# huzjkevin/planar_optical_flow

Measured on AMD Instinct MI355X. Metric: scans/sec, flow-only preprocess of 450-pt synthetic scan pairs, batch 4096 per GPU (+ flow EPE vs reference oracle), higher is better.
Workload: dtype f32 flow arithmetic (float32 outputs) + f64 exact association / mask decisions; the float64-output instantiation (the reference's float64 operation order) is `value_f64`

## Files before the change

planar_optical_flow_amd/csrc/scan_flow.hip:

```cpp
#include <cmath>
#include <cstdlib>
#include <type_traits>

#include "pof_common.h"

namespace {

constexpr int kThreads = 256;

__global__ void laser_phi_kernel(double start, double stop, double step, int n, double *tab)
{
    int i = blockIdx.x * blockDim.x + threadIdx.x;
    if (i >= n) return;
    double p = (double)i * step;
    p = p + start;
    if (i == n - 1 && n > 1) p = stop;
    double s, c;
    sincos(p, &s, &c);
    tab[i] = p;
    tab[n + 2 * i] = c;
    tab[n + 2 * i + 1] = s;
}

struct PreArgs {
    const float *ranges;
    long long sample_stride;
    int B, N, D;
    const double *tab;
    const double *odom0, *odom1;
    int flow_kind, canonical;
    void *xy, *flow;
    const int32_t *det_offsets;
    const double *det_rphi;
    const uint8_t *det_cls;
    double ra0, ra1, ra2;
    double sd0, sd1, sd2;
    double sa0, sa1, sa2;
    int32_t lb0, lb1, lb2;
    int64_t *closest, *target_cls;
    float *target_reg, *dyn_mask, *valid_mask, *exclude_mask;
    double *ws_rec;
    double *ws_det;
};

constexpr int kDetStride = 6;
constexpr int kInline = 8;
constexpr int kRecImg = 8 + kInline * kDetStride;
constexpr int kRecHdrFloats = 16;
constexpr int kImgScreen = kRecHdrFloats * 4;
constexpr int kImgCtr = kImgScreen + 16 * kInline;
constexpr int kImgMot = kImgCtr + 16 * kInline;
constexpr int kImgBytes = kImgMot + 64;
constexpr int kRecStride = kRecImg + kImgBytes / 8;

__device__ __forceinline__ double opaque_zero()
{
    double z;
    asm volatile("v_mov_b64 %0, 0" : "=v"(z));
    return z;
}

__device__ __forceinline__ void motion_params(int kind, const double *o0, const double *o1, double sA, double cA,
                              double sB, double cB, double *mot)
{
    const double tx = o1[0] - o0[0], ty = o1[1] - o0[1];
    if (kind == 0) {
        const float c0 = (float)cA, s0 = (float)sA, c1 = (float)cB, s1 = (float)sB;
        const float p00 = fmaf(s0, s1, c0 * c1);
        const float p01 = fmaf(s0, c1, c0 * (-s1));
        const float p10 = fmaf(c0, s1, (-s0) * c1);
        const float p11 = fmaf(c0, c1, (-s0) * (-s1));
        mot[0] = 1.0 - (double)p00;
        mot[1] = 0.0 - (double)p01;
        mot[2] = 0.0 - (double)p10;
        mot[3] = 1.0 - (double)p11;
        mot[4] = fma((double)c0, tx, (double)s0 * ty);
        mot[5] = fma((double)(-s0), tx, (double)c0 * ty);
        mot[6] = opaque_zero();
    } else if (kind == 1) {
        mot[0] = cB; mot[1] = -sB; mot[2] = sB; mot[3] = cB;
        mot[4] = fma(ty, -sA, tx * cA);
        mot[5] = fma(ty, cA, tx * sA);
        mot[6] = opaque_zero();
    } else if (kind == 2) {
        const float c1 = (float)cB, s1 = (float)sB;
        mot[0] = mot[1] = mot[2] = mot[3] = opaque_zero();
        mot[4] = fma((double)c1, tx, (double)s1 * ty);
        mot[5] = fma((double)(-s1), tx, (double)c1 * ty);
        mot[6] = o1[2] - o0[2];
    } else if (kind == 3) {
        const double dt = o1[0], den = dt + 1e-6;
        mot[0] = o0[2] / den;
        mot[1] = o0[0] / den;
        mot[2] = o0[1] / den;
        mot[3] = dt;
        mot[4] = mot[5] = mot[6] = opaque_zero();
    } else {
        const float c = (float)cA, sn = (float)sA, cd = (float)cB, sd = (float)sB;
        mot[0] = (double)c; mot[1] = (double)sn; mot[2] = (double)(-sn); mot[3] = (double)c;
        mot[4] = fma(o0[1], (double)(-sd), o0[0] * (double)cd);
        mot[5] = fma(o0[1], (double)cd, o0[0] * (double)sd);
        mot[6] = opaque_zero();
    }
}

__device__ __forceinline__ double motion_angle(int kind, int which, const double *o0, const double *o1)
{
    if (kind == 1) return which ? o1[2] - o0[2] : o0[2];
    if (kind == 4) return which ? o1[0] : o0[2];
    return which ? o1[2] : o0[2];
}

__device__ __forceinline__ void apply_motion(int kind, double px, double py, double m0, double m1, double m2,
                                             double m3, double t0, double t1, double dph, double &fx,
                                             double &fy)
{
    if (kind == 0) {
        fx = fma(py, m1, px * m0) - t0;
        fy = fma(py, m3, px * m2) - t1;
    } else if (kind == 1) {
        fx = (fma(py, m1, px * m0) - t0) - px;
        fy = (fma(py, m3, px * m2) - t1) - py;
    } else if (kind == 2) {
        fx = -t0 - (py * -dph);
        fy = -t1 - (px * dph);
    } else if (kind == 3) {
        fx = ((0.0 - m0 * py) + m1) * m3;
        fy = ((m0 * px - 0.0) + m2) * m3;
    } else {
        fx = fma(py, m1, px * m0) + t0;
        fy = fma(py, m3, px * m2) + t1;
    }
}

__device__ __forceinline__ double poly_sin(double x, double y)
{
    const double S1 = -1.66666666666666324348e-01, S2 = 8.33333333332248946124e-03, S3 = -1.98412698298579493134e-04,
                 S4 = 2.75573137070700676789e-06, S5 = -2.50507602534068634195e-08, S6 = 1.58969099521155010221e-10;
    const double z = x * x, v = z * x;
    const double r = S2 + z * (S3 + z * (S4 + z * (S5 + z * S6)));
    return x - ((z * (0.5 * y - v * r) - y) - v * S1);
}
__device__ __forceinline__ double poly_cos(double x, double y)
{
    const double C1 = 4.16666666666666019037e-02, C2 = -1.38888888888741095749e-03, C3 = 2.48015872894767294178e-05,
                 C4 = -2.75573143513906633035e-07, C5 = 2.08757232129817482790e-09, C6 = -1.13596475577881948265e-11;
    const double z = x * x;
    const double r = z * (C1 + z * (C2 + z * (C3 + z * (C4 + z * (C5 + z * C6)))));
    const double ax = fabs(x);
    if (ax < 0.3) return 1.0 - (0.5 * z - (z * r - x * y));
    const double qx = ax > 0.78125 ? 0.28125 : 0.25 * ax;
    const double hz = 0.5 * z - qx, a = 1.0 - qx;
    return a - (hz - (z * r - x * y));
}
template <bool FALLBACK>
__device__ __forceinline__ void params_sincos(double x, double *sn, double *cs)
{
    const double ax = fabs(x);
    if (!(ax < 823549.0)) {
        if (FALLBACK) {
            sincos(x, sn, cs);
        } else {
            *sn = *cs = __builtin_nan("");
// ... 14 lines not shown
        r = t - w;
        w = fn * p2t - ((t - r) - w);
        y0 = r - w;
        if (ex - ((__double2hiint(y0) >> 20) & 0x7ff) > 49) {
            t = r;
            w = fn * p3;
            r = t - w;
            w = fn * p3t - ((t - r) - w);
            y0 = r - w;
        }
    }
    double y1 = (r - y0) - w;
    int n = (int)fn;
    if (x < 0.0) {
        y0 = -y0;
        y1 = -y1;
        n = -n;
    }
    const double s = poly_sin(y0, y1), c = poly_cos(y0, y1);
    const bool odd = (n & 1) != 0;
    double ss = odd ? c : s, cc = odd ? s : c;
    if (n & 2) ss = -ss;
    if ((n + 1) & 2) cc = -cc;
    *sn = ss;
    *cs = cc;
}

template <typename AP>
__device__ __forceinline__ void det_entry(AP a, int g, double *w)
{
    const double dr = a->det_rphi[2 * g], dp = a->det_rphi[2 * g + 1];
    double s, c;
    sincos(dp, &s, &c);
    const int cl = a->det_cls[g];
    w[0] = dr * c;
    w[1] = dr * s;
    w[2] = cl == 0 ? a->ra0 : (cl == 1 ? a->ra1 : a->ra2);
    w[3] = cl == 0 ? a->sd0 : (cl == 1 ? a->sd1 : a->sd2);
    w[4] = (double)(cl == 0 ? a->lb0 : (cl == 1 ? a->lb1 : a->lb2));
    w[5] = cl == 0 ? a->sa0 : (cl == 1 ? a->sa1 : a->sa2);
}

__device__ __forceinline__ bool det_is_far(double cx, double cy, double sd)
{
    return !(fabs(cx) + fabs(cy) < 100.0) || !(sd <= 400.0);
}

__host__ __device__ inline int params_job_count(int B, bool have_dets)
{
    (void)have_dets;
    return kInline * B;
}

template <bool FALLBACK, bool WRITE_F64, typename AP>
__device__ __forceinline__ void params_work(AP a, int t)
{
    if (t >= kInline * a->B) return;
    const int b = t >> 3, slot = t & 7;
    double *rec = a->ws_rec + (long long)b * kRecStride;
    unsigned char *img = reinterpret_cast<unsigned char *>(rec + kRecImg);
    int d0 = 0, cnt = 0;
    if (a->det_offsets) {
        d0 = a->det_offsets[b];
        cnt = a->det_offsets[b + 1] - d0;
    }
    const int npass = 1 + (cnt - slot + kInline - 1) / kInline;
#pragma unroll 1
    for (int pass = a->flow ? 0 : 1; pass < max(npass, 1); ++pass) {
        const int idx = slot + kInline * (pass - 1);
        const bool active = pass == 0 ? slot < 2 : idx < cnt;
        double ang = 0.0, dr = 0.0;
        if (pass == 0) {
            if (active) ang = motion_angle(a->flow_kind, slot, a->odom0 + 3 * b, a->odom1 + 3 * b);
        } else if (active) {
            dr = a->det_rphi[2 * (d0 + idx)];
            ang = a->det_rphi[2 * (d0 + idx) + 1];
        }
        double sn, cs;
        params_sincos<FALLBACK>(ang, &sn, &cs);
        if (pass == 0) {
            const double s_o = __shfl_xor(sn, 1, 64), c_o = __shfl_xor(cs, 1, 64);
            if (slot == 0) {
                double *m64 = reinterpret_cast<double *>(img + kImgMot);
                motion_params(a->flow_kind, a->odom0 + 3 * b, a->odom1 + 3 * b, sn, cs, s_o, c_o, m64);
                m64[7] = (double)cnt;
                float4 *hf = reinterpret_cast<float4 *>(img);
                hf[0] = make_float4((float)m64[0], (float)m64[1], (float)m64[2], (float)m64[3]);
                hf[1] = make_float4((float)m64[4], (float)m64[5], (float)m64[6], __int_as_float(cnt));
                if (WRITE_F64) {
                    double2 *r2 = reinterpret_cast<double2 *>(rec);
#pragma unroll
                    for (int k = 0; k < 4; ++k) r2[k] = make_double2(m64[2 * k], m64[2 * k + 1]);
                }
            }
        } else if (active) {
            const unsigned cl = a->det_cls[d0 + idx] > 1 ? 2u : (unsigned)a->det_cls[d0 + idx];
            double w[kDetStride];
            w[0] = dr * cs;
            w[1] = dr * sn;
            w[2] = cl == 0 ? a->ra0 : (cl == 1 ? a->ra1 : a->ra2);
            w[3] = cl == 0 ? a->sd0 : (cl == 1 ? a->sd1 : a->sd2);
            w[4] = (double)(cl == 0 ? a->lb0 : (cl == 1 ? a->lb1 : a->lb2));
            w[5] = cl == 0 ? a->sa0 : (cl == 1 ? a->sa1 : a->sa2);
            if (idx < kInline) {
                const bool far = det_is_far(w[0], w[1], w[3]);
                reinterpret_cast<float4 *>(img + kImgScreen)[idx] =
                    make_float4((float)w[0], (float)w[1], far ? INFINITY : -(float)w[3], (float)(w[5] - w[3]));
                reinterpret_cast<double2 *>(img + kImgCtr)[idx] = make_double2(w[0], w[1]);
                img[32 + idx] = (unsigned char)cl;
                img[40 + idx] = far ? 1 : 0;
                if (WRITE_F64) {
                    double2 *r2 = reinterpret_cast<double2 *>(rec + 8 + idx * kDetStride);
                    r2[0] = make_double2(w[0], w[1]);
                    r2[1] = make_double2(w[2], w[3]);
                    r2[2] = make_double2(w[4], w[5]);
                }
            }
            if (cnt > kInline) {
                double2 *r2 = reinterpret_cast<double2 *>(a->ws_det + (long long)(d0 + idx) * kDetStride);
                r2[0] = make_double2(w[0], w[1]);
                r2[1] = make_double2(w[2], w[3]);
                r2[2] = make_double2(w[4], w[5]);
            }
        }
    }
    if (!a->flow && slot == 0) {
        reinterpret_cast<int *>(img)[7] = cnt;
        reinterpret_cast<double *>(img + kImgMot)[7] = (double)cnt;
        if (WRITE_F64) rec[7] = (double)cnt;
    }
    if (a->det_offsets && slot >= cnt) {
        reinterpret_cast<float4 *>(img + kImgScreen)[slot] = make_float4(0.0f, 0.0f, INFINITY, 0.0f);
        img[40 + slot] = 0;
    }
}

__global__ __launch_bounds__(256) void scan_params_kernel(PreArgs a)
{
    params_work<true, true>(&a, blockIdx.x * blockDim.x + threadIdx.x);
}

__device__ __forceinline__ double to_sgpr(double v)
{
    const int lo = __builtin_amdgcn_readfirstlane(__double2loint(v));
    const int hi = __builtin_amdgcn_readfirstlane(__double2hiint(v));
    return __hiloint2double(hi, lo);
}

#define GLOBAL_AS __attribute__((address_space(1)))
using F4V = float __attribute__((ext_vector_type(4)));
using F2V = float __attribute__((ext_vector_type(2)));
using LL2V = long long __attribute__((ext_vector_type(2)));
__device__ __forceinline__ void stream_f4(float *base, long long idx4, float x, float y, float z, float w)
{
    F4V v = {x, y, z, w};
    __builtin_nontemporal_store(v, (GLOBAL_AS F4V *)base + idx4);
}
__device__ __forceinline__ void stream_f2(float *base, long long idx2, float x, float y)
{
    F2V v = {x, y};
    __builtin_nontemporal_store(v, (GLOBAL_AS F2V *)base + idx2);
}
__device__ __forceinline__ void stream_ll2(long long *base, long long idx2, long long x, long long y)
{
    LL2V v = {x, y};
    __builtin_nontemporal_store(v, (GLOBAL_AS LL2V *)base + idx2);
}

template <typename OutT>
__device__ __forceinline__ void store2(OutT *base, long long idx, double a, double b)
{
    using V = OutT __attribute__((ext_vector_type(2)));
    V v = {(OutT)a, (OutT)b};
    ((GLOBAL_AS V *)base)[idx] = v;
}

constexpr int kDetTile = 32;

__device__ __forceinline__ float4 prefilter_entry(double cx, double cy, double sd, double sa)
{
    const bool far = !(fabs(cx) + fabs(cy) < 100.0);
    return make_float4((float)cx, (float)cy, (float)sd, far ? INFINITY : (float)sa);
// ... 293 lines not shown
    FlatBatch b[kMaxSlots];
};

struct ParamsMulti {
    int nb;
    int first, total;
    int uni_blocks;
    unsigned uni_m;
    int uni_s;
    int blk0[kMaxSlots + 1];
    PreArgs p[kMaxSlots];
};

template <typename T>
__device__ __forceinline__ T fma_t(T a, T b, T c);
template <>
__device__ __forceinline__ double fma_t<double>(double a, double b, double c) { return fma(a, b, c); }
template <>
__device__ __forceinline__ float fma_t<float>(float a, float b, float c) { return fmaf(a, b, c); }

template <typename T>
__device__ __forceinline__ void apply_motion_t(int kind, T px, T py, T m0, T m1, T m2, T m3, T t0, T t1, T dph,
                                               T &fx, T &fy)
{
    if (kind == 0) {
        fx = fma_t<T>(py, m1, px * m0) - t0;
        fy = fma_t<T>(py, m3, px * m2) - t1;
    } else if (kind == 1) {
        fx = (fma_t<T>(py, m1, px * m0) - t0) - px;
        fy = (fma_t<T>(py, m3, px * m2) - t1) - py;
    } else if (kind == 2) {
        fx = -t0 - (py * -dph);
        fy = -t1 - (px * dph);
    } else if (kind == 3) {
        fx = ((T)0 - m0 * py + m1) * m3;
        fy = ((m0 * px - (T)0) + m2) * m3;
    } else {
        fx = fma_t<T>(py, m1, px * m0) + t0;
        fy = fma_t<T>(py, m3, px * m2) + t1;
    }
}

template <int CFG>
struct FlatCfg {
    unsigned rt;
    __device__ __forceinline__ bool has(unsigned bit) const { return CFG >= 0 ? ((unsigned)CFG & bit) != 0 : (rt & bit) != 0; }
    __device__ __forceinline__ int kind() const { return CFG >= 0 ? (CFG >> kKindShift) & 7 : (int)(rt >> kKindShift) & 7; }
};

using D2V = double __attribute__((ext_vector_type(2)));

struct RunLoads {
    float2 rv;
    float4 tf;
    D2V t0v, t1v;
    int local, q;
    bool ok;
};

template <typename OutT>
__device__ __forceinline__ RunLoads flat_loads(const FlatArgs &L, const FlatBatch &bt, const int lane, const int sA,
                                               const int l0)
{
    constexpr bool kF32 = sizeof(OutT) == 4;
    RunLoads in;
    int local = l0 + lane;
    const int q = local >= L.halfN ? 1 : 0;
    local -= q ? L.halfN : 0;
    in.local = local;
    in.q = q;
    in.ok = sA + q < bt.B;
    const unsigned i0 = 2u * (unsigned)local;
    const GLOBAL_AS float *rowA = (const GLOBAL_AS float *)bt.ranges + (long long)sA * bt.sample_stride;
    const unsigned roff = (q && in.ok ? (unsigned)bt.sample_stride : 0u) + i0;
    const F2V rr = *(const GLOBAL_AS F2V *)(rowA + roff);
    in.rv = make_float2(rr.x, rr.y);
    in.tf = make_float4(0.f, 0.f, 0.f, 0.f);
    in.t0v = D2V{0.0, 0.0};
    in.t1v = D2V{0.0, 0.0};
    if (kF32 && L.tabf) {
        in.tf = *reinterpret_cast<const float4 *>(L.tabf + 2u * i0);
    } else {
        const double *tab_cs = L.tab + L.N;
        in.t0v = *reinterpret_cast<const D2V *>(tab_cs + 2u * i0);
        in.t1v = *reinterpret_cast<const D2V *>(tab_cs + 2u * i0 + 2);
    }
    return in;
}

template <typename OutT, int CFG>
__device__ __forceinline__ void flat_run(const FlatArgs &L, const FlatBatch &bt, const FlatCfg<CFG> cfg,
                                         const unsigned char *lds, const int lane, const int sA, const int l0,
                                         const long long pair0, const RunLoads &in)
{
    constexpr bool kF32 = sizeof(OutT) == 4;
    const int halfN = L.halfN, N = L.N;
    const int local = in.local, q = in.q;
    const int b = sA + q;
    const bool ok = in.ok;
    const int i0 = 2 * local;
    const float2 rv = in.rv;
    const double *tab_cs = L.tab + N;
    float csf[2], snf[2];
    const D2V t0v = in.t0v, t1v = in.t1v;
    if (kF32 && L.tabf) {
        csf[0] = in.tf.x; snf[0] = in.tf.y; csf[1] = in.tf.z; snf[1] = in.tf.w;
    } else {
        csf[0] = (float)t0v.x; snf[0] = (float)t0v.y; csf[1] = (float)t1v.x; snf[1] = (float)t1v.y;
    }
    const float r[2] = {rv.x, rv.y};
    F2V pxf = {r[0] * csf[0], r[1] * csf[1]}, pyf = {r[0] * snf[0], r[1] * snf[1]};
    auto cs64 = [&](int k) { return tab_cs[2u * (unsigned)(i0 + k)]; };
    auto sn64 = [&](int k) { return tab_cs[2u * (unsigned)(i0 + k) + 1]; };
    auto p64x = [&](int k) { return (double)r[k] * cs64(k); };
    auto p64y = [&](int k) { return (double)r[k] * sn64(k); };
    const unsigned char *hdr = lds + q * kImgBytes;

    if (cfg.has(kOutXy) && ok) {
        OutT *xy = static_cast<OutT *>(bt.xy) + 4 * pair0;
        store2<OutT>(xy, 2u * (unsigned)lane, p64x(0), p64y(0));
        store2<OutT>(xy, 2u * (unsigned)lane + 1, p64x(1), p64y(1));
    }

    if (cfg.has(kOutFlow)) {
        const int kind = cfg.kind();
        if (kF32 && kind != 1) {
            const float4 ma = *reinterpret_cast<const float4 *>(hdr);
            const float4 mb = *reinterpret_cast<const float4 *>(hdr + 16);
            float fxs[2], fys[2];
#pragma unroll
            for (int k = 0; k < 2; ++k) {
                float fx, fy;
                apply_motion_t<float>(kind, pxf[k], pyf[k], ma.x, ma.y, ma.z, ma.w, mb.x, mb.y, mb.z, fx, fy);
                if (cfg.has(kCanonical)) {
                    const float gx = fmaf(csf[k], fx, -snf[k] * fy);
                    const float gy = fmaf(snf[k], fx, csf[k] * fy);
                    fx = gx;
                    fy = gy;
                }
                fxs[k] = fx;
                fys[k] = fy;
            }
            if (ok) stream_f4(reinterpret_cast<float *>(bt.flow) + 4 * pair0, (unsigned)lane, fxs[0], fys[0], fxs[1], fys[1]);
        } else {
            const double *mot = reinterpret_cast<const double *>(hdr + kImgMot);
            const double m0 = mot[0], m1 = mot[1], m2 = mot[2], m3 = mot[3];
            const double tr0 = mot[4], tr1 = mot[5], dph = mot[6];
            OutT *fl = static_cast<OutT *>(bt.flow) + 4 * pair0;
            double cs[2], sn[2];
            if (kF32 && L.tabf) {
                cs[0] = cs64(0); sn[0] = sn64(0); cs[1] = cs64(1); sn[1] = sn64(1);
            } else {
                cs[0] = t0v.x; sn[0] = t0v.y; cs[1] = t1v.x; sn[1] = t1v.y;
            }
            double f[4];
#pragma unroll
            for (int k = 0; k < 2; ++k) {
                double fx, fy;
                apply_motion(kind, (double)r[k] * cs[k], (double)r[k] * sn[k], m0, m1, m2, m3, tr0, tr1, dph, fx, fy);
                if (cfg.has(kCanonical)) {
                    const double gx = cs[k] * fx + (-sn[k]) * fy;
                    const double gy = sn[k] * fx + cs[k] * fy;
                    fx = gx;
                    fy = gy;
                }
                f[2 * k] = fx;
                f[2 * k + 1] = fy;
            }
            if (ok) {
                if (kF32) {
                    stream_f4(reinterpret_cast<float *>(fl), (unsigned)lane, (float)f[0], (float)f[1], (float)f[2], (float)f[3]);
                } else {
                    D2V v0 = {f[0], f[1]}, v1 = {f[2], f[3]};
                    GLOBAL_AS D2V *dst = (GLOBAL_AS D2V *)fl + 2u * (unsigned)lane;
                    __builtin_nontemporal_store(v0, dst);
                    __builtin_nontemporal_store(v1, dst + 1);
                }
            }
        }
    }

    float vmask[2], dmask[2];
#pragma unroll
    for (int k = 0; k < 2; ++k) {
        vmask[k] = (r[k] >= 20.0f) ? 0.0f : 1.0f;
        dmask[k] = 1.0f;
    }

    if (cfg.has(kHasDets)) {
        const bool want_assoc = cfg.has(kOutClosest) || cfg.has(kOutCls) || cfg.has(kOutReg);
        const bool want_dyn = cfg.has(kOutDyn) || cfg.has(kOutExcl);
        const int4 h1 = *reinterpret_cast<const int4 *>(hdr + 16);
        const int2 h2 = *reinterpret_cast<const int2 *>(hdr + 32);
        const int2 h3 = *reinterpret_cast<const int2 *>(hdr + 40);
        const int nd = ok ? h1.w : 0;
        const int n_in = min(nd, kInline);
        const int nA = l0 < halfN ? reinterpret_cast<const int *>(lds)[7] : 0;
        const int nB = l0 + 63 >= halfN ? reinterpret_cast<const int *>(lds + kImgBytes)[7] : 0;
        const int n_loop = __builtin_amdgcn_readfirstlane(min(max(nA, nB), kInline));
        F2V mind = {INFINITY, INFINITY};
        const unsigned char *ent = hdr + kImgScreen;
        for (int j = 0; j < n_loop; ++j) {
            const float4 e = *reinterpret_cast<const float4 *>(ent + 16 * j);
            const F2V cx2 = {e.x, e.x}, cy2 = {e.y, e.y}, ns2 = {e.z, e.z};
            const F2V ex = pxf - cx2, ey = pyf - cy2;
            F2V d = __builtin_elementwise_fma(ey, ey, ns2);
            d = __builtin_elementwise_fma(ex, ex, d);
            mind = __builtin_elementwise_min(mind, d);
        }
        const bool samp_far = (h3.x | h3.y) != 0;
        int bidx[2] = {0, 0};
        int dfirst = 0;
        auto cls_of = [&](int j) { return ((j < 4 ? h2.x : h2.y) >> (8 * (j & 3))) & 3; };
        auto sel3 = [&](const double *v, int c) { return c == 0 ? v[0] : (c == 1 ? v[1] : v[2]); };
        auto candidate = [&](int k, int j1, double s2, double ra) {
            if (bidx[k] != 0) {
                double wx, wy, wra;
                if (bidx[k] <= kInline) {
                    const D2V c = *reinterpret_cast<const D2V *>(hdr + kImgCtr + 16 * (bidx[k] - 1));
                    wx = c.x; wy = c.y; wra = sel3(L.ra, cls_of(bidx[k] - 1));
                } else {
                    const GLOBAL_AS double *w = (const GLOBAL_AS double *)bt.ws_det + (long long)(dfirst + bidx[k] - 1) * kDetStride;
                    wx = w[0]; wy = w[1]; wra = w[2];
                }
                const double exd = p64x(k) - wx, eyd = p64y(k) - wy;
                if (!(sqrt(s2) - ra < sqrt(exd * exd + eyd * eyd) - wra)) return;
            }
            bidx[k] = j1;
        };
#pragma unroll
        for (int k = 0; k < 2; ++k) {
            const bool exk = samp_far || !(fabsf(pxf[k]) + fabsf(pyf[k]) < 100.0f);
            bool need_dyn = false;
            if (!exk && mind[k] <= -L.m_dyn) dmask[k] = 0.0f;
            else need_dyn = want_dyn && (exk || mind[k] <= L.m_dyn);
            bool need_assoc = want_assoc && (exk || mind[k] <= L.thr_assoc);
            if (need_assoc && !exk) {
                int ncand = 0, jc = 0;
                bool unsure = false;
                for (int j = 0; j < n_in; ++j) {
                    const float4 e = *reinterpret_cast<const float4 *>(ent + 16 * j);
                    const float exf = pxf[k] - e.x, eyf = pyf[k] - e.y;
                    const float d = fmaf(exf, exf, fmaf(eyf, eyf, e.z));
                    if (d <= e.w + L.m_assoc) {
                        if (d <= e.w - L.m_assoc) { ++ncand; jc = j; }
                        else unsure = true;
                    }
                }
                if (!unsure && ncand <= 1) {
                    if (ncand == 1) bidx[k] = jc + 1;
                    need_assoc = false;
                }
            }
            if (need_dyn || need_assoc) {
                const double pxd = p64x(k), pyd = p64y(k);
                for (int j = 0; j < n_in; ++j) {
                    const D2V c = *reinterpret_cast<const D2V *>(hdr + kImgCtr + 16 * j);
                    const int cl = cls_of(j);
                    const double exd = pxd - c.x, eyd = pyd - c.y;
                    const double s2 = exd * exd + eyd * eyd;
                    if (need_dyn && s2 <= sel3(L.sd, cl)) dmask[k] = 0.0f;
                    if (need_assoc && s2 <= sel3(L.sa, cl)) candidate(k, j + 1, s2, sel3(L.ra, cl));
                }
            }
        }
        if (nd > kInline) {
            dfirst = ((const GLOBAL_AS int32_t *)bt.det_offsets)[b];
            for (int j = kInline; j < nd; ++j) {
                const GLOBAL_AS double *w = (const GLOBAL_AS double *)bt.ws_det + (long long)(dfirst + j) * kDetStride;
                const double cx = w[0], cy = w[1], ra = w[2], sd = w[3], sa = w[5];
#pragma unroll
                for (int k = 0; k < 2; ++k) {
                    const double exd = p64x(k) - cx, eyd = p64y(k) - cy;
                    const double s2 = exd * exd + eyd * eyd;
                    if (s2 <= sd) dmask[k] = 0.0f;
                    if (want_assoc && s2 <= sa) candidate(k, j + 1, s2, ra);
                }
            }
        }
        if (ok && want_assoc) {
            long long cls[2];
            float gx[2], gy[2];
#pragma unroll
            for (int k = 0; k < 2; ++k) {
                cls[k] = 0;
                gx[k] = gy[k] = 0.0f;
                if (bidx[k] > 0) {
                    double wx, wy;
                    if (bidx[k] <= kInline) {
                        const D2V c = *reinterpret_cast<const D2V *>(hdr + kImgCtr + 16 * (bidx[k] - 1));
                        wx = c.x; wy = c.y;
                        const int cl = cls_of(bidx[k] - 1);
                        cls[k] = cl == 0 ? L.lb[0] : (cl == 1 ? L.lb[1] : L.lb[2]);
                    } else {
                        const GLOBAL_AS double *w = (const GLOBAL_AS double *)bt.ws_det + (long long)(dfirst + bidx[k] - 1) * kDetStride;
                        wx = w[0];
                        wy = w[1];
                        cls[k] = (long long)w[4];
                    }
                    const double c = cs64(k), sn_ = sn64(k);
                    gx[k] = (float)(wy * c - wx * sn_);
                    gy[k] = (float)((wx * c + wy * sn_) - (double)r[k]);
                }
            }
            if (cfg.has(kOutClosest)) stream_ll2(reinterpret_cast<long long *>(bt.closest) + 2 * pair0, (unsigned)lane, bidx[0], bidx[1]);
            if (cfg.has(kOutCls)) stream_ll2(reinterpret_cast<long long *>(bt.target_cls) + 2 * pair0, (unsigned)lane, cls[0], cls[1]);
            if (cfg.has(kOutReg)) stream_f4(bt.target_reg + 4 * pair0, (unsigned)lane, gx[0], gy[0], gx[1], gy[1]);
        }
    }

    if (ok) {
        if (cfg.has(kOutDyn)) stream_f2(bt.dyn_mask + 2 * pair0, (unsigned)lane, dmask[0], dmask[1]);
        if (cfg.has(kOutValid)) stream_f2(bt.valid_mask + 2 * pair0, (unsigned)lane, vmask[0], vmask[1]);
        if (cfg.has(kOutExcl)) stream_f2(bt.exclude_mask + 2 * pair0, (unsigned)lane, dmask[0] * vmask[0], dmask[1] * vmask[1]);
    }
}

typedef const __attribute__((address_space(4))) unsigned char *kernarg_ptr;
template <typename S>
__device__ __forceinline__ S kernarg_struct(kernarg_ptr p)
{
    static_assert(sizeof(S) % 8 == 0, "kernarg slots are read in 8-byte words");
    S out;
    unsigned long long *w = reinterpret_cast<unsigned long long *>(&out);
#pragma unroll
    for (int i = 0; i < (int)(sizeof(S) / 8); ++i)
        w[i] = *reinterpret_cast<const __attribute__((address_space(4))) unsigned long long *>(p + 8 * i);
    return out;
}
constexpr size_t kFlatArgsKernargBytes = (sizeof(FlatArgs) + 7) & ~(size_t)7;

template <typename OutT, int CFG, int THREADS, int CPW>
__global__ __launch_bounds__(THREADS, 8) void scan_flat_kernel(const FlatArgs L, const ParamsMulti P)
{
    constexpr int WAVES = THREADS / 64;
    __shared__ __align__(16) unsigned char smem[WAVES][kWaveLds];
    kernarg_ptr ka = (kernarg_ptr)__builtin_amdgcn_kernarg_segment_ptr();
    int sblock = (int)blockIdx.x;
    if (sblock >= P.first) {
        if (sblock < P.first + P.total) {
#ifndef POF_FLAT_NO_PARAMS
            const int blk = sblock - P.first;
            int k = 0, b0 = P.blk0[0];
            if (P.uni_blocks) {
                k = (int)(__umulhi((unsigned)blk, P.uni_m) >> P.uni_s);
                b0 = k * P.uni_blocks;
            } else {
#pragma unroll
                for (int i = 1; i < kMaxSlots; ++i) k += (blk >= P.blk0[i]) ? 1 : 0;
                k = __builtin_amdgcn_readfirstlane(k);
#pragma unroll
                for (int i = 1; i < kMaxSlots; ++i) b0 = (k >= i) ? P.blk0[i] : b0;
            }
            const auto *pa = reinterpret_cast<const __attribute__((address_space(4))) PreArgs *>(
                ka + kFlatArgsKernargBytes + offsetof(ParamsMulti, p) + (size_t)k * sizeof(PreArgs));
            params_work<false, false>(pa, (blk - b0) * THREADS + (int)threadIdx.x);
#endif
            return;
        }
        sblock -= P.total;
    }
    const int wv = __builtin_amdgcn_readfirstlane((int)threadIdx.x >> 6);
    const int lane = (int)threadIdx.x & 63;
    const int w = sblock * WAVES + wv;
    if (w >= L.total_waves) return;
    int k = 0;
    if (L.uni_waves) {
        k = (int)(__umulhi((unsigned)w, L.uni_m) >> L.uni_s);
    } else {
#pragma unroll
        for (int i = 1; i < kMaxSlots; ++i) k += (w >= L.wave0[i]) ? 1 : 0;
    }
    k = __builtin_amdgcn_readfirstlane(k);
    const FlatBatch bt = kernarg_struct<FlatBatch>(ka + offsetof(FlatArgs, b) + (size_t)k * sizeof(FlatBatch));
    const FlatCfg<CFG> cfg{L.flags};
    unsigned char *lds = smem[wv];

    const unsigned p0 = (unsigned)(w - bt.wave0) * (64u * CPW);
    const int sA = (int)(__umulhi(p0, L.magic_m) >> L.magic_s);
    const int l0 = (int)(p0 - (unsigned)sA * (unsigned)L.halfN);

    RunLoads in[CPW];
#pragma unroll
    for (int c = 0; c < CPW; ++c) in[c] = flat_loads<OutT>(L, bt, lane, sA, l0 + 64 * c);

    if (cfg.has(kOutFlow) || cfg.has(kHasDets)) {
        {
            const int sq = lane >> 5, i = lane & 31;
            if (i < kImgBytes / 16) {
                const double *rec = bt.ws_rec + (long long)min(sA + sq, bt.B - 1) * kRecStride;
                *reinterpret_cast<F4V *>(lds + sq * kImgBytes + 16 * i) = ((const GLOBAL_AS F4V *)(rec + kRecImg))[i];
            }
        }
        __builtin_amdgcn_fence(__ATOMIC_RELEASE, "wavefront");
        __builtin_amdgcn_wave_barrier();
        __builtin_amdgcn_fence(__ATOMIC_ACQUIRE, "wavefront");
    }
#pragma unroll
    for (int c = 0; c < CPW; ++c)
        flat_run<OutT, CFG>(L, bt, cfg, lds, lane, sA, l0 + 64 * c, (long long)p0 + 64 * c, in[c]);
}

template <typename T>
__global__ void rotate_flow_kernel(const T *in, T *out, const double *tab, long long total, int N,
                                   int to_canonical)
{
    long long p = (long long)blockIdx.x * blockDim.x + threadIdx.x;
    if (p >= total) return;
    int i = (int)(p % N);
    double c = tab[N + 2 * i], s = tab[N + 2 * i + 1];
    double fx = (double)in[2 * p], fy = (double)in[2 * p + 1];
    double gx, gy;
    if (to_canonical) {
        gx = c * fx + (-s) * fy;
// ... 629 lines not shown
```

Before: 397.6 million.

## Restructure params prologue and streaming loads to reuse f64 trig table values

Restructures params_work so that odometry and detection inputs are loaded up front, with detections software-prefetched one iteration ahead, and the motion header is written once at the end as double2 stores. In the streaming kernel, the f32 trig table path is removed: cos/sin are always read once from the f64 table and reused for both the float and double computations, replacing repeated global re-reads in the lambdas. The detection association loop is merged and moved ahead of the flow output. This is meant to cut redundant global loads and improve load/store vectorization, at the cost of reading wider f64 table entries on the f32 path.

```diff
diff --git a/planar_optical_flow_amd/csrc/scan_flow.hip b/planar_optical_flow_amd/csrc/scan_flow.hip
--- a/planar_optical_flow_amd/csrc/scan_flow.hip
+++ b/planar_optical_flow_amd/csrc/scan_flow.hip
@@ -60,55 +60,88 @@
     return z;
 }
 
-__device__ __forceinline__ void motion_params(int kind, const double *o0, const double *o1, double sA, double cA,
-                              double sB, double cB, double *mot)
-{
-    const double tx = o1[0] - o0[0], ty = o1[1] - o0[1];
-    if (kind == 0) {
+struct Motion {
+    double m0, m1, m2, m3, m4, m5, m6;
+};
+struct Odom {
+    double x, y, z;
+};
+
+__device__ __forceinline__ Motion motion_values(int kind, const Odom o0, const Odom o1, double sA, double cA, double sB,
+                                                double cB)
+{
+    Motion m;
+    switch (kind) {
+    case 0: {
+        const double tx = o1.x - o0.x, ty = o1.y - o0.y;
         const float c0 = (float)cA, s0 = (float)sA, c1 = (float)cB, s1 = (float)sB;
         const float p00 = fmaf(s0, s1, c0 * c1);
         const float p01 = fmaf(s0, c1, c0 * (-s1));
         const float p10 = fmaf(c0, s1, (-s0) * c1);
         const float p11 = fmaf(c0, c1, (-s0) * (-s1));
-        mot[0] = 1.0 - (double)p00;
-        mot[1] = 0.0 - (double)p01;
-        mot[2] = 0.0 - (double)p10;
-        mot[3] = 1.0 - (double)p11;
-        mot[4] = fma((double)c0, tx, (double)s0 * ty);
-        mot[5] = fma((double)(-s0), tx, (double)c0 * ty);
-        mot[6] = opaque_zero();
-    } else if (kind == 1) {
-        mot[0] = cB; mot[1] = -sB; mot[2] = sB; mot[3] = cB;
-        mot[4] = fma(ty, -sA, tx * cA);
-        mot[5] = fma(ty, cA, tx * sA);
-        mot[6] = opaque_zero();
-    } else if (kind == 2) {
+        m.m0 = 1.0 - (double)p00;
+        m.m1 = 0.0 - (double)p01;
+        m.m2 = 0.0 - (double)p10;
+        m.m3 = 1.0 - (double)p11;
+        m.m4 = fma((double)c0, tx, (double)s0 * ty);
+        m.m5 = fma((double)(-s0), tx, (double)c0 * ty);
+        m.m6 = opaque_zero();
+        break;
+    }
+    case 1: {
+        const double tx = o1.x - o0.x, ty = o1.y - o0.y;
+        m.m0 = cB; m.m1 = -sB; m.m2 = sB; m.m3 = cB;
+        m.m4 = fma(ty, -sA, tx * cA);
+        m.m5 = fma(ty, cA, tx * sA);
+        m.m6 = opaque_zero();
+        break;
+    }
+    case 2: {
+        const double tx = o1.x - o0.x, ty = o1.y - o0.y;
         const float c1 = (float)cB, s1 = (float)sB;
-        mot[0] = mot[1] = mot[2] = mot[3] = opaque_zero();
-        mot[4] = fma((double)c1, tx, (double)s1 * ty);
-        mot[5] = fma((double)(-s1), tx, (double)c1 * ty);
-        mot[6] = o1[2] - o0[2];
-    } else if (kind == 3) {
-        const double dt = o1[0], den = dt + 1e-6;
-        mot[0] = o0[2] / den;
-        mot[1] = o0[0] / den;
-        mot[2] = o0[1] / den;
-        mot[3] = dt;
-        mot[4] = mot[5] = mot[6] = opaque_zero();
-    } else {
+        m.m0 = m.m1 = m.m2 = m.m3 = opaque_zero();
+        m.m4 = fma((double)c1, tx, (double)s1 * ty);
+        m.m5 = fma((double)(-s1), tx, (double)c1 * ty);
+        m.m6 = o1.z - o0.z;
+        break;
+    }
+    case 3: {
+        const double dt = o1.x, den = dt + 1e-6;
+        m.m0 = o0.z / den;
+        m.m1 = o0.x / den;
+        m.m2 = o0.y / den;
+        m.m3 = dt;
+        m.m4 = m.m5 = m.m6 = opaque_zero();
+        break;
+    }
+    default: {
         const float c = (float)cA, sn = (float)sA, cd = (float)cB, sd = (float)sB;
-        mot[0] = (double)c; mot[1] = (double)sn; mot[2] = (double)(-sn); mot[3] = (double)c;
-        mot[4] = fma(o0[1], (double)(-sd), o0[0] * (double)cd);
-        mot[5] = fma(o0[1], (double)cd, o0[0] * (double)sd);
-        mot[6] = opaque_zero();
-    }
-}
-
+        m.m0 = (double)c; m.m1 = (double)sn; m.m2 = (double)(-sn); m.m3 = (double)c;
+        m.m4 = fma(o0.y, (double)(-sd), o0.x * (double)cd);
+        m.m5 = fma(o0.y, (double)cd, o0.x * (double)sd);
+        m.m6 = opaque_zero();
+        break;
+    }
+    }
+    return m;
+}
+
+__device__ __forceinline__ void motion_params(int kind, const double *o0, const double *o1, double sA, double cA,
+                              double sB, double cB, double *mot)
+{
+    const Motion m = motion_values(kind, Odom{o0[0], o0[1], o0[2]}, Odom{o1[0], o1[1], o1[2]}, sA, cA, sB, cB);
+    mot[0] = m.m0; mot[1] = m.m1; mot[2] = m.m2; mot[3] = m.m3; mot[4] = m.m4; mot[5] = m.m5; mot[6] = m.m6;
+}
+
+__device__ __forceinline__ double motion_angle(int kind, int which, const Odom o0, const Odom o1)
+{
+    if (kind == 1) return which ? o1.z - o0.z : o0.z;
+    if (kind == 4) return which ? o1.x : o0.z;
+    return which ? o1.z : o0.z;
+}
 __device__ __forceinline__ double motion_angle(int kind, int which, const double *o0, const double *o1)
 {
-    if (kind == 1) return which ? o1[2] - o0[2] : o0[2];
-    if (kind == 4) return which ? o1[0] : o0[2];
-    return which ? o1[2] : o0[2];
+    return motion_angle(kind, which, Odom{o0[0], o0[1], o0[2]}, Odom{o1[0], o1[1], o1[2]});
 }
 
 __device__ __forceinline__ void apply_motion(int kind, double px, double py, double m0, double m1, double m2,
@@ -229,82 +262,123 @@
     return kInline * B;
 }
 
+typedef const __attribute__((address_space(4))) PreArgs *PreArgsKernarg;
+__device__ __forceinline__ const PreArgs *loop_local(const PreArgs *a) { return a; }
+__device__ __forceinline__ PreArgsKernarg loop_local(PreArgsKernarg a)
+{
+    asm volatile("" : "+s"(a));
+    return a;
+}
+
 template <bool FALLBACK, bool WRITE_F64, typename AP>
 __device__ __forceinline__ void params_work(AP a, int t)
 {
     if (t >= kInline * a->B) return;
     const int b = t >> 3, slot = t & 7;
-    double *rec = a->ws_rec + (long long)b * kRecStride;
-    unsigned char *img = reinterpret_cast<unsigned char *>(rec + kRecImg);
+    double *__restrict__ rec = a->ws_rec + (long long)b * kRecStride;
+    unsigned char *__restrict__ img = reinterpret_cast<unsigned char *>(rec + kRecImg);
+    const bool has_flow = a->flow != nullptr;
+    const int kind = a->flow_kind;
+
+    Odom o0 = {0.0, 0.0, 0.0}, o1 = {0.0, 0.0, 0.0};
+    if (has_flow) {
+        const double *__restrict__ p0 = a->odom0 + 3 * b, *__restrict__ p1 = a->odom1 + 3 * b;
+        o0 = Odom{p0[0], p0[1], p0[2]};
+        o1 = Odom{p1[0], p1[1], p1[2]};
+    }
     int d0 = 0, cnt = 0;
     if (a->det_offsets) {
-        d0 = a->det_offsets[b];
-        cnt = a->det_offsets[b + 1] - d0;
-    }
-    const int npass = 1 + (cnt - slot + kInline - 1) / kInline;
-#pragma unroll 1
-    for (int pass = a->flow ? 0 : 1; pass < max(npass, 1); ++pass) {
-        const int idx = slot + kInline * (pass - 1);
-        const bool active = pass == 0 ? slot < 2 : idx < cnt;
-        double ang = 0.0, dr = 0.0;
-        if (pass == 0) {
-            if (active) ang = motion_angle(a->flow_kind, slot, a->odom0 + 3 * b, a->odom1 + 3 * b);
-        } else if (active) {
-            dr = a->det_rphi[2 * (d0 + idx)];
-            ang = a->det_rphi[2 * (d0 + idx) + 1];
-        }
+        const int32_t *__restrict__ offs = a->det_offsets;
+        d0 = offs[b];
+        cnt = offs[b + 1] - d0;
+    }
+    struct DetIn {
+        double r, ang;
+        unsigned cl;
+    };
+    auto fetch = [&](int idx) {
+        DetIn d = {0.0, 0.0, 0u};
+        if (idx < cnt) {
+            const double *__restrict__ rp = a->det_rphi + 2 * (long long)(d0 + idx);
+            d.r = rp[0];
+            d.ang = rp[1];
+            d.cl = a->det_cls[d0 + idx];
+        }
+        return d;
+    };
+    DetIn nx = fetch(slot);
+
+    Motion mot = {0.0, 0.0, 0.0, 0.0, 0.0, 0.0, 0.0};
+    if (has_flow) {
+        const double ang = slot < 2 ? motion_angle(kind, slot, o0, o1) : 0.0;
         double sn, cs;
         params_sincos<FALLBACK>(ang, &sn, &cs);
-        if (pass == 0) {
-            const double s_o = __shfl_xor(sn, 1, 64), c_o = __shfl_xor(cs, 1, 64);
-            if (slot == 0) {
-                double *m64 = reinterpret_cast<double *>(img + kImgMot);
-                motion_params(a->flow_kind, a->odom0 + 3 * b, a->odom1 + 3 * b, sn, cs, s_o, c_o, m64);
-                m64[7] = (double)cnt;
-                float4 *hf = reinterpret_cast<float4 *>(img);
-                hf[0] = make_float4((float)m64[0], (float)m64[1], (float)m64[2], (float)m64[3]);
-                hf[1] = make_float4((float)m64[4], (float)m64[5], (float)m64[6], __int_as_float(cnt));
-                if (WRITE_F64) {
-                    double2 *r2 = reinterpret_cast<double2 *>(rec);
-#pragma unroll
-                    for (int k = 0; k < 4; ++k) r2[k] = make_double2(m64[2 * k], m64[2 * k + 1]);
-                }
-            }
-        } else if (active) {
-            const unsigned cl = a->det_cls[d0 + idx] > 1 ? 2u : (unsigned)a->det_cls[d0 + idx];
-            double w[kDetStride];
-            w[0] = dr * cs;
-            w[1] = dr * sn;
-            w[2] = cl == 0 ? a->ra0 : (cl == 1 ? a->ra1 : a->ra2);
-            w[3] = cl == 0 ? a->sd0 : (cl == 1 ? a->sd1 : a->sd2);
-            w[4] = (double)(cl == 0 ? a->lb0 : (cl == 1 ? a->lb1 : a->lb2));
-            w[5] = cl == 0 ? a->sa0 : (cl == 1 ? a->sa1 : a->sa2);
-            if (idx < kInline) {
-                const bool far = det_is_far(w[0], w[1], w[3]);
-                reinterpret_cast<float4 *>(img + kImgScreen)[idx] =
-                    make_float4((float)w[0], (float)w[1], far ? INFINITY : -(float)w[3], (float)(w[5] - w[3]));
-                reinterpret_cast<double2 *>(img + kImgCtr)[idx] = make_double2(w[0], w[1]);
-                img[32 + idx] = (unsigned char)cl;
-                img[40 + idx] = far ? 1 : 0;
-                if (WRITE_F64) {
-                    double2 *r2 = reinterpret_cast<double2 *>(rec + 8 + idx * kDetStride);
-                    r2[0] = make_double2(w[0], w[1]);
-                    r2[1] = make_double2(w[2], w[3]);
-                    r2[2] = make_double2(w[4], w[5]);
-                }
-            }
-            if (cnt > kInline) {
-                double2 *r2 = reinterpret_cast<double2 *>(a->ws_det + (long long)(d0 + idx) * kDetStride);
+        const double s_o = __shfl_xor(sn, 1, 64), c_o = __shfl_xor(cs, 1, 64);
+        if (slot == 0) mot = motion_values(kind, o0, o1, sn, cs, s_o, c_o);
+    }
+
+#pragma unroll 1
+    for (int idx = slot; idx < cnt; idx += kInline) {
+        const DetIn cur = nx;
+        nx = fetch(idx + kInline);
+        double sn, cs;
+        params_sincos<FALLBACK>(cur.ang, &sn, &cs);
+        const unsigned cl = cur.cl > 1 ? 2u : cur.cl;
+        const auto al = loop_local(a);
+        const double ra0 = al->ra0, ra1 = al->ra1, ra2 = al->ra2, sd0 = al->sd0, sd1 = al->sd1, sd2 = al->sd2;
+        const double sa0 = al->sa0, sa1 = al->sa1, sa2 = al->sa2;
+        const int lb0 = al->lb0, lb1 = al->lb1, lb2 = al->lb2;
+        double w[kDetStride];
+        w[0] = cur.r * cs;
+        w[1] = cur.r * sn;
+        w[2] = cl == 0 ? ra0 : (cl == 1 ? ra1 : ra2);
+        w[3] = cl == 0 ? sd0 : (cl == 1 ? sd1 : sd2);
+        w[4] = (double)(cl == 0 ? lb0 : (cl == 1 ? lb1 : lb2));
+        w[5] = cl == 0 ? sa0 : (cl == 1 ? sa1 : sa2);
+        if (idx < kInline) {
+            const bool far = det_is_far(w[0], w[1], w[3]);
+            reinterpret_cast<float4 *>(img + kImgScreen)[idx] =
+                make_float4((float)w[0], (float)w[1], far ? INFINITY : -(float)w[3], (float)(w[5] - w[3]));
+            reinterpret_cast<double2 *>(img + kImgCtr)[idx] = make_double2(w[0], w[1]);
+            img[32 + idx] = (unsigned char)cl;
+            img[40 + idx] = far ? 1 : 0;
+            if (WRITE_F64) {
+                double2 *r2 = reinterpret_cast<double2 *>(rec + 8 + idx * kDetStride);
                 r2[0] = make_double2(w[0], w[1]);
                 r2[1] = make_double2(w[2], w[3]);
                 r2[2] = make_double2(w[4], w[5]);
             }
         }
-    }
-    if (!a->flow && slot == 0) {
-        reinterpret_cast<int *>(img)[7] = cnt;
-        reinterpret_cast<double *>(img + kImgMot)[7] = (double)cnt;
-        if (WRITE_F64) rec[7] = (double)cnt;
+        if (cnt > kInline) {
+            double2 *r2 = reinterpret_cast<double2 *>(a->ws_det + (long long)(d0 + idx) * kDetStride);
+            r2[0] = make_double2(w[0], w[1]);
+            r2[1] = make_double2(w[2], w[3]);
+            r2[2] = make_double2(w[4], w[5]);
+        }
+    }
+
+    if (slot == 0) {
+        if (has_flow) {
+            float4 *hf = reinterpret_cast<float4 *>(img);
+            hf[0] = make_float4((float)mot.m0, (float)mot.m1, (float)mot.m2, (float)mot.m3);
+            hf[1] = make_float4((float)mot.m4, (float)mot.m5, (float)mot.m6, __int_as_float(cnt));
+            double2 *m2 = reinterpret_cast<double2 *>(img + kImgMot);
+            m2[0] = make_double2(mot.m0, mot.m1);
+            m2[1] = make_double2(mot.m2, mot.m3);
+            m2[2] = make_double2(mot.m4, mot.m5);
+            m2[3] = make_double2(mot.m6, (double)cnt);
+            if (WRITE_F64) {
+                double2 *r2 = reinterpret_cast<double2 *>(rec);
+                r2[0] = make_double2(mot.m0, mot.m1);
+                r2[1] = make_double2(mot.m2, mot.m3);
+                r2[2] = make_double2(mot.m4, mot.m5);
+                r2[3] = make_double2(mot.m6, (double)cnt);
+            }
+        } else {
+            reinterpret_cast<int *>(img)[7] = cnt;
+            reinterpret_cast<double *>(img + kImgMot)[7] = (double)cnt;
+            if (WRITE_F64) rec[7] = (double)cnt;
+        }
     }
     if (a->det_offsets && slot >= cnt) {
         reinterpret_cast<float4 *>(img + kImgScreen)[slot] = make_float4(0.0f, 0.0f, INFINITY, 0.0f);
@@ -704,7 +778,6 @@
 
 struct RunLoads {
     float2 rv;
-    float4 tf;
     D2V t0v, t1v;
     int local, q;
     bool ok;
@@ -714,7 +787,6 @@
 __device__ __forceinline__ RunLoads flat_loads(const FlatArgs &L, const FlatBatch &bt, const int lane, const int sA,
                                                const int l0)
 {
-    constexpr bool kF32 = sizeof(OutT) == 4;
     RunLoads in;
     int local = l0 + lane;
     const int q = local >= L.halfN ? 1 : 0;
@@ -727,16 +799,9 @@
     const unsigned roff = (q && in.ok ? (unsigned)bt.sample_stride : 0u) + i0;
     const F2V rr = *(const GLOBAL_AS F2V *)(rowA + roff);
     in.rv = make_float2(rr.x, rr.y);
-    in.tf = make_float4(0.f, 0.f, 0.f, 0.f);
-    in.t0v = D2V{0.0, 0.0};
-    in.t1v = D2V{0.0, 0.0};
-    if (kF32 && L.tabf) {
-        in.tf = *reinterpret_cast<const float4 *>(L.tabf + 2u * i0);
-    } else {
-        const double *tab_cs = L.tab + L.N;
-        in.t0v = *reinterpret_cast<const D2V *>(tab_cs + 2u * i0);
-        in.t1v = *reinterpret_cast<const D2V *>(tab_cs + 2u * i0 + 2);
-    }
+    const double *tab_cs = L.tab + L.N;
+    in.t0v = *reinterpret_cast<const D2V *>(tab_cs + 2u * i0);
+    in.t1v = *reinterpret_cast<const D2V *>(tab_cs + 2u * i0 + 2);
     return in;
 }
 
@@ -746,104 +811,30 @@
                                          const long long pair0, const RunLoads &in)
 {
     constexpr bool kF32 = sizeof(OutT) == 4;
-    const int halfN = L.halfN, N = L.N;
-    const int local = in.local, q = in.q;
+    const int halfN = L.halfN;
+    const int q = in.q;
     const int b = sA + q;
     const bool ok = in.ok;
-    const int i0 = 2 * local;
     const float2 rv = in.rv;
-    const double *tab_cs = L.tab + N;
-    float csf[2], snf[2];
-    const D2V t0v = in.t0v, t1v = in.t1v;
-    if (kF32 && L.tabf) {
-        csf[0] = in.tf.x; snf[0] = in.tf.y; csf[1] = in.tf.z; snf[1] = in.tf.w;
-    } else {
-        csf[0] = (float)t0v.x; snf[0] = (float)t0v.y; csf[1] = (float)t1v.x; snf[1] = (float)t1v.y;
-    }
+    const D2V c64[2] = {in.t0v, in.t1v};
+    const float csf[2] = {(float)c64[0].x, (float)c64[1].x}, snf[2] = {(float)c64[0].y, (float)c64[1].y};
     const float r[2] = {rv.x, rv.y};
     F2V pxf = {r[0] * csf[0], r[1] * csf[1]}, pyf = {r[0] * snf[0], r[1] * snf[1]};
-    auto cs64 = [&](int k) { return tab_cs[2u * (unsigned)(i0 + k)]; };
-    auto sn64 = [&](int k) { return tab_cs[2u * (unsigned)(i0 + k) + 1]; };
+    auto cs64 = [&](int k) { return c64[k].x; };
+    auto sn64 = [&](int k) { return c64[k].y; };
     auto p64x = [&](int k) { return (double)r[k] * cs64(k); };
     auto p64y = [&](int k) { return (double)r[k] * sn64(k); };
     const unsigned char *hdr = lds + q * kImgBytes;
 
-    if (cfg.has(kOutXy) && ok) {
-        OutT *xy = static_cast<OutT *>(bt.xy) + 4 * pair0;
-        store2<OutT>(xy, 2u * (unsigned)lane, p64x(0), p64y(0));
-        store2<OutT>(xy, 2u * (unsigned)lane + 1, p64x(1), p64y(1));
-    }
-
-    if (cfg.has(kOutFlow)) {
-        const int kind = cfg.kind();
-        if (kF32 && kind != 1) {
-            const float4 ma = *reinterpret_cast<const float4 *>(hdr);
-            const float4 mb = *reinterpret_cast<const float4 *>(hdr + 16);
-            float fxs[2], fys[2];
-#pragma unroll
-            for (int k = 0; k < 2; ++k) {
-                float fx, fy;
-                apply_motion_t<float>(kind, pxf[k], pyf[k], ma.x, ma.y, ma.z, ma.w, mb.x, mb.y, mb.z, fx, fy);
-                if (cfg.has(kCanonical)) {
-                    const float gx = fmaf(csf[k], fx, -snf[k] * fy);
-                    const float gy = fmaf(snf[k], fx, csf[k] * fy);
-                    fx = gx;
-                    fy = gy;
-                }
-                fxs[k] = fx;
-                fys[k] = fy;
-            }
-            if (ok) stream_f4(reinterpret_cast<float *>(bt.flow) + 4 * pair0, (unsigned)lane, fxs[0], fys[0], fxs[1], fys[1]);
-        } else {
-            const double *mot = reinterpret_cast<const double *>(hdr + kImgMot);
-            const double m0 = mot[0], m1 = mot[1], m2 = mot[2], m3 = mot[3];
-            const double tr0 = mot[4], tr1 = mot[5], dph = mot[6];
-            OutT *fl = static_cast<OutT *>(bt.flow) + 4 * pair0;
-            double cs[2], sn[2];
-            if (kF32 && L.tabf) {
-                cs[0] = cs64(0); sn[0] = sn64(0); cs[1] = cs64(1); sn[1] = sn64(1);
-            } else {
-                cs[0] = t0v.x; sn[0] = t0v.y; cs[1] = t1v.x; sn[1] = t1v.y;
-            }
-            double f[4];
-#pragma unroll
-            for (int k = 0; k < 2; ++k) {
-                double fx, fy;
-                apply_motion(kind, (double)r[k] * cs[k], (double)r[k] * sn[k], m0, m1, m2, m3, tr0, tr1, dph, fx, fy);
-                if (cfg.has(kCanonical)) {
-                    const double gx = cs[k] * fx + (-sn[k]) * fy;
-                    const double gy = sn[k] * fx + cs[k] * fy;
-                    fx = gx;
-                    fy = gy;
-                }
-                f[2 * k] = fx;
-                f[2 * k + 1] = fy;
-            }
-            if (ok) {
-                if (kF32) {
-                    stream_f4(reinterpret_cast<float *>(fl), (unsigned)lane, (float)f[0], (float)f[1], (float)f[2], (float)f[3]);
-                } else {
-                    D2V v0 = {f[0], f[1]}, v1 = {f[2], f[3]};
-                    GLOBAL_AS D2V *dst = (GLOBAL_AS D2V *)fl + 2u * (unsigned)lane;
-                    __builtin_nontemporal_store(v0, dst);
-                    __builtin_nontemporal_store(v1, dst + 1);
-                }
-            }
-        }
-    }
-
-    float vmask[2], dmask[2];
-#pragma unroll
-    for (int k = 0; k < 2; ++k) {
-        vmask[k] = (r[k] >= 20.0f) ? 0.0f : 1.0f;
-        dmask[k] = 1.0f;
-    }
+    bool dyn_hit[2] = {false, false};
+    int best[2] = {0, 0};
+    int cls[2] = {0, 0};
+    float gx[2] = {0.0f, 0.0f}, gy[2] = {0.0f, 0.0f};
 
     if (cfg.has(kHasDets)) {
         const bool want_assoc = cfg.has(kOutClosest) || cfg.has(kOutCls) || cfg.has(kOutReg);
         const bool want_dyn = cfg.has(kOutDyn) || cfg.has(kOutExcl);
         const int4 h1 = *reinterpret_cast<const int4 *>(hdr + 16);
-        const int2 h2 = *reinterpret_cast<const int2 *>(hdr + 32);
         const int2 h3 = *reinterpret_cast<const int2 *>(hdr + 40);
         const int nd = ok ? h1.w : 0;
         const int n_in = min(nd, kInline);
@@ -863,10 +854,11 @@
         const bool samp_far = (h3.x | h3.y) != 0;
         int bidx[2] = {0, 0};
         int dfirst = 0;
-        auto cls_of = [&](int j) { return ((j < 4 ? h2.x : h2.y) >> (8 * (j & 3))) & 3; };
+        auto cls_of = [&](int j) { return (int)hdr[32 + j] & 3; };
         auto sel3 = [&](const double *v, int c) { return c == 0 ? v[0] : (c == 1 ? v[1] : v[2]); };
-        auto candidate = [&](int k, int j1, double s2, double ra) {
+        auto candidate = [&](int k, int j1, double s2, auto ra_of) {
             if (bidx[k] != 0) {
+                const double lhs = sqrt(s2) - ra_of();
                 double wx, wy, wra;
                 if (bidx[k] <= kInline) {
                     const D2V c = *reinterpret_cast<const D2V *>(hdr + kImgCtr + 16 * (bidx[k] - 1));
@@ -876,17 +868,24 @@
                     wx = w[0]; wy = w[1]; wra = w[2];
                 }
                 const double exd = p64x(k) - wx, eyd = p64y(k) - wy;
-                if (!(sqrt(s2) - ra < sqrt(exd * exd + eyd * eyd) - wra)) return;
+                if (!(lhs < sqrt(exd * exd + eyd * eyd) - wra)) return;
             }
             bidx[k] = j1;
         };
+        bool exk2[2], need_dyn2[2], need_assoc2[2];
 #pragma unroll
         for (int k = 0; k < 2; ++k) {
-            const bool exk = samp_far || !(fabsf(pxf[k]) + fabsf(pyf[k]) < 100.0f);
-            bool need_dyn = false;
-            if (!exk && mind[k] <= -L.m_dyn) dmask[k] = 0.0f;
-            else need_dyn = want_dyn && (exk || mind[k] <= L.m_dyn);
-            bool need_assoc = want_assoc && (exk || mind[k] <= L.thr_assoc);
+            exk2[k] = samp_far || !(fabsf(pxf[k]) + fabsf(pyf[k]) < 100.0f);
+            need_dyn2[k] = false;
+            if (!exk2[k] && mind[k] <= -L.m_dyn) dyn_hit[k] = true;
+            else need_dyn2[k] = want_dyn && (exk2[k] || mind[k] <= L.m_dyn);
+            need_assoc2[k] = want_assoc && (exk2[k] || mind[k] <= L.thr_assoc);
+        }
+        if (nd > kInline) dfirst = ((const GLOBAL_AS int32_t *)bt.det_offsets)[b];
+#pragma unroll
+        for (int k = 0; k < 2; ++k) {
+            const bool exk = exk2[k], need_dyn = need_dyn2[k];
+            bool need_assoc = need_assoc2[k];
             if (need_assoc && !exk) {
                 int ncand = 0, jc = 0;
                 bool unsure = false;
@@ -904,64 +903,131 @@
                     need_assoc = false;
                 }
             }
-            if (need_dyn || need_assoc) {
+            const int jbeg = (need_dyn || need_assoc) ? 0 : kInline;
+            if (jbeg < nd) {
                 const double pxd = p64x(k), pyd = p64y(k);
-                for (int j = 0; j < n_in; ++j) {
-                    const D2V c = *reinterpret_cast<const D2V *>(hdr + kImgCtr + 16 * j);
-                    const int cl = cls_of(j);
-                    const double exd = pxd - c.x, eyd = pyd - c.y;
+#pragma unroll 1
+                for (int j = jbeg; j < nd; ++j) {
+                    const bool inl = j < kInline;
+                    double cx, cy, sd, sa;
+                    if (inl) {
+                        const D2V c = *reinterpret_cast<const D2V *>(hdr + kImgCtr + 16 * j);
+                        const int cl = cls_of(j);
+                        cx = c.x; cy = c.y;
+                        sd = sel3(L.sd, cl); sa = sel3(L.sa, cl);
+                    } else {
+                        const GLOBAL_AS double *w = (const GLOBAL_AS double *)bt.ws_det + (long long)(dfirst + j) * kDetStride;
+                        cx = w[0]; cy = w[1]; sd = w[3]; sa = w[5];
+                    }
+                    auto ra_of = [&]() {
+                        return inl ? sel3(L.ra, cls_of(j))
+                                   : ((const GLOBAL_AS double *)bt.ws_det + (long long)(dfirst + j) * kDetStride)[2];
+                    };
+                    const double exd = pxd - cx, eyd = pyd - cy;
                     const double s2 = exd * exd + eyd * eyd;
-                    if (need_dyn && s2 <= sel3(L.sd, cl)) dmask[k] = 0.0f;
-                    if (need_assoc && s2 <= sel3(L.sa, cl)) candidate(k, j + 1, s2, sel3(L.ra, cl));
+                    if ((need_dyn || !inl) && s2 <= sd) dyn_hit[k] = true;
+                    if ((inl ? need_assoc : want_assoc) && s2 <= sa) candidate(k, j + 1, s2, ra_of);
                 }
             }
-        }
-        if (nd > kInline) {
-            dfirst = ((const GLOBAL_AS int32_t *)bt.det_offsets)[b];
-            for (int j = kInline; j < nd; ++j) {
-                const GLOBAL_AS double *w = (const GLOBAL_AS double *)bt.ws_det + (long long)(dfirst + j) * kDetStride;
-                const double cx = w[0], cy = w[1], ra = w[2], sd = w[3], sa = w[5];
-#pragma unroll
-                for (int k = 0; k < 2; ++k) {
-                    const double exd = p64x(k) - cx, eyd = p64y(k) - cy;
-                    const double s2 = exd * exd + eyd * eyd;
-                    if (s2 <= sd) dmask[k] = 0.0f;
-                    if (want_assoc && s2 <= sa) candidate(k, j + 1, s2, ra);
+            if (ok && want_assoc && bidx[k] > 0) {
+                double wx, wy;
+                if (bidx[k] <= kInline) {
+                    const D2V c = *reinterpret_cast<const D2V *>(hdr + kImgCtr + 16 * (bidx[k] - 1));
+                    wx = c.x; wy = c.y;
+                    const int cl = cls_of(bidx[k] - 1);
+                    cls[k] = cl == 0 ? L.lb[0] : (cl == 1 ? L.lb[1] : L.lb[2]);
+                } else {
+                    const GLOBAL_AS double *w = (const GLOBAL_AS double *)bt.ws_det + (long long)(dfirst + bidx[k] - 1) * kDetStride;
+                    wx = w[0];
+                    wy = w[1];
+                    cls[k] = (int)w[4];
                 }
-            }
-        }
-        if (ok && want_assoc) {
-            long long cls[2];
-            float gx[2], gy[2];
+                const double c = cs64(k), sn_ = sn64(k);
+                gx[k] = (float)(wy * c - wx * sn_);
+                gy[k] = (float)((wx * c + wy * sn_) - (double)r[k]);
+            }
+        }
+        best[0] = bidx[0];
+        best[1] = bidx[1];
+    }
+
+    if (cfg.has(kOutXy) && ok) {
+        OutT *xy = static_cast<OutT *>(bt.xy) + 4 * pair0;
+        store2<OutT>(xy, 2u * (unsigned)lane, p64x(0), p64y(0));
+        store2<OutT>(xy, 2u * (unsigned)lane + 1, p64x(1), p64y(1));
+    }
+
+    float ff[4] = {0.f, 0.f, 0.f, 0.f};
+    double fd[4] = {0.0, 0.0, 0.0, 0.0};
+    if (cfg.has(kOutFlow)) {
+        const int kind = cfg.kind();
+        if (kF32 && kind != 1) {
+            const float4 ma = *reinterpret_cast<const float4 *>(hdr);
+            const float4 mb = *reinterpret_cast<const float4 *>(hdr + 16);
+            float fxs[2], fys[2];
 #pragma unroll
             for (int k = 0; k < 2; ++k) {
-                cls[k] = 0;
-                gx[k] = gy[k] = 0.0f;
-                if (bidx[k] > 0) {
-                    double wx, wy;
-                    if (bidx[k] <= kInline) {
-                        const D2V c = *reinterpret_cast<const D2V *>(hdr + kImgCtr + 16 * (bidx[k] - 1));
-                        wx = c.x; wy = c.y;
-                        const int cl = cls_of(bidx[k] - 1);
-                        cls[k] = cl == 0 ? L.lb[0] : (cl == 1 ? L.lb[1] : L.lb[2]);
-                    } else {
-                        const GLOBAL_AS double *w = (const GLOBAL_AS double *)bt.ws_det + (long long)(dfirst + bidx[k] - 1) * kDetStride;
-                        wx = w[0];
-                        wy = w[1];
-                        cls[k] = (long long)w[4];
-                    }
-                    const double c = cs64(k), sn_ = sn64(k);
-                    gx[k] = (float)(wy * c - wx * sn_);
-                    gy[k] = (float)((wx * c + wy * sn_) - (double)r[k]);
+                float fx, fy;
+                apply_motion_t<float>(kind, pxf[k], pyf[k], ma.x, ma.y, ma.z, ma.w, mb.x, mb.y, mb.z, fx, fy);
+                if (cfg.has(kCanonical)) {
+                    const float gx_ = fmaf(csf[k], fx, -snf[k] * fy);
+                    const float gy_ = fmaf(snf[k], fx, csf[k] * fy);
+                    fx = gx_;
+                    fy = gy_;
                 }
-            }
-            if (cfg.has(kOutClosest)) stream_ll2(reinterpret_cast<long long *>(bt.closest) + 2 * pair0, (unsigned)lane, bidx[0], bidx[1]);
-            if (cfg.has(kOutCls)) stream_ll2(reinterpret_cast<long long *>(bt.target_cls) + 2 * pair0, (unsigned)lane, cls[0], cls[1]);
+                fxs[k] = fx;
+                fys[k] = fy;
+            }
+            ff[0] = fxs[0]; ff[1] = fys[0]; ff[2] = fxs[1]; ff[3] = fys[1];
+        } else {
+            const double *mot = reinterpret_cast<const double *>(hdr + kImgMot);
+            const double m0 = mot[0], m1 = mot[1], m2 = mot[2], m3 = mot[3];
+            const double tr0 = mot[4], tr1 = mot[5], dph = mot[6];
+            const double cs[2] = {cs64(0), cs64(1)}, sn[2] = {sn64(0), sn64(1)};
+            double f[4];
+#pragma unroll
+            for (int k = 0; k < 2; ++k) {
+                double fx, fy;
+                apply_motion(kind, (double)r[k] * cs[k], (double)r[k] * sn[k], m0, m1, m2, m3, tr0, tr1, dph, fx, fy);
+                if (cfg.has(kCanonical)) {
+                    const double gx_ = cs[k] * fx + (-sn[k]) * fy;
+                    const double gy_ = sn[k] * fx + cs[k] * fy;
+                    fx = gx_;
+                    fy = gy_;
+                }
+                f[2 * k] = fx;
+                f[2 * k + 1] = fy;
+            }
+            if (kF32) {
+                ff[0] = (float)f[0]; ff[1] = (float)f[1]; ff[2] = (float)f[2]; ff[3] = (float)f[3];
+            } else {
+                fd[0] = f[0]; fd[1] = f[1]; fd[2] = f[2]; fd[3] = f[3];
+            }
+        }
+    }
+
+    if (cfg.has(kOutFlow) && ok) {
+        if (kF32) {
+            stream_f4(reinterpret_cast<float *>(bt.flow) + 4 * pair0, (unsigned)lane, ff[0], ff[1], ff[2], ff[3]);
+        } else {
+            D2V v0 = {fd[0], fd[1]}, v1 = {fd[2], fd[3]};
+            GLOBAL_AS D2V *dst = (GLOBAL_AS D2V *)(static_cast<OutT *>(bt.flow) + 4 * pair0) + 2u * (unsigned)lane;
+            __builtin_nontemporal_store(v0, dst);
+            __builtin_nontemporal_store(v1, dst + 1);
+        }
+    }
+    if (ok) {
+        if (cfg.has(kHasDets) && (cfg.has(kOutClosest) || cfg.has(kOutCls) || cfg.has(kOutReg))) {
+            if (cfg.has(kOutClosest)) stream_ll2(reinterpret_cast<long long *>(bt.closest) + 2 * pair0, (unsigned)lane, best[0], best[1]);
+            if (cfg.has(kOutCls)) stream_ll2(reinterpret_cast<long long *>(bt.target_cls) + 2 * pair0, (unsigned)lane, (long long)cls[0], (long long)cls[1]);
             if (cfg.has(kOutReg)) stream_f4(bt.target_reg + 4 * pair0, (unsigned)lane, gx[0], gy[0], gx[1], gy[1]);
         }
-    }
-
-    if (ok) {
+        float vmask[2], dmask[2];
+#pragma unroll
+        for (int k = 0; k < 2; ++k) {
+            vmask[k] = (r[k] >= 20.0f) ? 0.0f : 1.0f;
+            dmask[k] = dyn_hit[k] ? 0.0f : 1.0f;
+        }
         if (cfg.has(kOutDyn)) stream_f2(bt.dyn_mask + 2 * pair0, (unsigned)lane, dmask[0], dmask[1]);
         if (cfg.has(kOutValid)) stream_f2(bt.valid_mask + 2 * pair0, (unsigned)lane, vmask[0], vmask[1]);
         if (cfg.has(kOutExcl)) stream_f2(bt.exclude_mask + 2 * pair0, (unsigned)lane, dmask[0] * vmask[0], dmask[1] * vmask[1]);
@@ -1012,6 +1078,7 @@
         }
         sblock -= P.total;
     }
+    asm volatile("; pof-role: streaming");
     const int wv = __builtin_amdgcn_readfirstlane((int)threadIdx.x >> 6);
     const int lane = (int)threadIdx.x & 63;
     const int w = sblock * WAVES + wv;
```

Measured after the change: 400.9 million, median of 4. About the same (+0.8%).
